# satoken/ractip

Hardware: NVIDIA B200
Metric: shuffled pairs/sec, probability stage of --zscore=12 (McCaskill in/out x2 + unpaired windows x2 + two-strand McCaskill) (higher is better)
Workload: dtype f64

## Files before the change

### ractip_b200/csrc/mcc_band.h

```cpp
#ifndef RP_MCC_BAND_H
#define RP_MCC_BAND_H

#include "mcc_core.h"

namespace rp {

constexpr int BR = 8;
constexpr int BSLOTS = 32;
constexpr int NSLICE = 16;

struct SmallModel {
  double scale1, mlb1, expMLclosing, expMLintern, expTermAU, inv_expTermAU;
  double scale_small[10];
  double mmI[8][5][5], mmH[8][5][5], mmM[8][5][5], mmExt[8][5][5], mm1n[8][5][5];
  double dangle5[8][5], dangle3[8][5];
  const double* spw;
  int special_hp, pad;
};
constexpr int SM_DOUBLES = (int)((sizeof(SmallModel) + 7) / 8);

struct DiagDesc;
struct BandShared {
  int LDB, LD8;
  int NGP;
  double *TI, *T1, *TA;
  double* ipart;
  double *cI, *c1, *cA;
  double* G;
  double *gA, *g1;
  double* sIv;
  SmallModel* sm;
  DiagDesc* desc;
};
constexpr int GPACK = (MAXLOOP + 1) * (MAXLOOP + 2) / 2;
constexpr int DESC_DOUBLES = 4 * 6;

RP_HD int band_ldb(int n) { return ((n + 1 + 7) / 8) * 8; }
RP_HD int band_ngp(int n) { return (n + 7) / 8 + 3; }
#ifdef __CUDACC__
constexpr bool BAND_SHFL = true;
#else
constexpr bool BAND_SHFL = false;
#endif
RP_HD size_t band_part_doubles(int n, int T, bool shfl = BAND_SHFL) {
  const size_t a = shfl ? (size_t)2 * BAND * (32 - (BAND - 1)) * (T / 32) : (size_t)2 * BAND * T;
  const size_t b = (size_t)(NSLICE + 1) * BR * band_ngp(n);
  return a > b ? a : b;
}
RP_HD size_t band_shared_doubles(int n, int T, bool shfl = BAND_SHFL) {
  return band_part_doubles(n, T, shfl) + 128  + (size_t)3 * BSLOTS * band_ldb(n) + (size_t)3 * BR * band_ngp(n) +
         GPACK + 64 + (size_t)(n + 2) + SM_DOUBLES + DESC_DOUBLES + (size_t)(n + 2 + 7) / 8 + 2;
}
RP_HD size_t band_shared_bytes(int n, int T, bool shfl = BAND_SHFL) { return band_shared_doubles(n, T, shfl) * sizeof(double); }

RP_HD void carve_band(Shared& sh, BandShared& bs, void* base, int n, int T, bool shfl = BAND_SHFL) {
  sh.T = T;
  double* p = static_cast<double*>(base);
  sh.part = p; bs.ipart = p; p += band_part_doubles(n, T, shfl);
  sh.red = p; p += 128;
  bs.LDB = band_ldb(n); bs.LD8 = bs.LDB / 8; bs.NGP = band_ngp(n);
  bs.TI = p; p += (size_t)BSLOTS * bs.LDB;
  bs.T1 = p; p += (size_t)BSLOTS * bs.LDB;
  bs.TA = p; p += (size_t)BSLOTS * bs.LDB;
  bs.cI = p; p += (size_t)BR * bs.NGP;
  bs.c1 = p; p += (size_t)BR * bs.NGP;
  bs.cA = p; p += (size_t)BR * bs.NGP;
  bs.G = p; p += GPACK;
  bs.gA = p; p += 32;
  bs.g1 = p; p += 32;
  bs.sIv = p; p += n + 2;
  bs.sm = reinterpret_cast<SmallModel*>(p); p += SM_DOUBLES;
  bs.desc = reinterpret_cast<DiagDesc*>(p); p += DESC_DOUBLES;
  sh.S = reinterpret_cast<uint8_t*>(p);
  sh.grow = nullptr; sh.ghead_b = nullptr; sh.ghead_1 = nullptr;
}

RP_HD void load_band_weights(const DevModel& M, const BandShared& bs, int tid, int T) {
  for (int x = tid; x < GPACK; x += T) bs.G[x] = M.gpack[x];
  for (int s = tid; s < 32; s += T) { bs.gA[s] = M.gA[s]; bs.g1[s] = M.g1[s]; }
  SmallModel& S = *bs.sm;
  if (tid == 0) {
    S.scale1 = M.scale1; S.mlb1 = M.mlb1; S.expMLclosing = M.expMLclosing; S.expMLintern = M.expMLintern;
    S.expTermAU = M.expTermAU; S.inv_expTermAU = 1.0 / M.expTermAU;
    for (int k = 0; k < 10; k++) S.scale_small[k] = M.scale_small[k];
    S.spw = M.spw;
    S.special_hp = M.special_hp; S.pad = 0;
  }
  for (int x = tid; x < 200; x += T) {
    (&S.mmI[0][0][0])[x] = (&M.mmI[0][0][0])[x];
    (&S.mmH[0][0][0])[x] = (&M.mmH[0][0][0])[x];
    (&S.mmM[0][0][0])[x] = (&M.mmM[0][0][0])[x];
    (&S.mmExt[0][0][0])[x] = (&M.mmExt[0][0][0])[x];
    (&S.mm1n[0][0][0])[x] = (&M.mm1n[0][0][0])[x];
    if (x < 40) {
      (&S.dangle5[0][0])[x] = (&M.dangle5[0][0])[x];
      (&S.dangle3[0][0])[x] = (&M.dangle3[0][0])[x];
    }
  }
}

RP_HD int bidx(const BandShared& bs, int p) { return (p & 7) * bs.LD8 + (p >> 3); }
RP_HD double* brow(double* band, const BandShared& bs, int d) { return band + (size_t)(d & (BSLOTS - 1)) * bs.LDB; }

struct Segs {
  int b[4];
  int G[4];
};
RP_HD Segs make_segs(int n, int cp, int d, bool cross_only = false) {
  Segs s;
  const int C = n - d;
  s.b[0] = 1; s.b[3] = C + 1;
  if (cp <= 0) { s.b[1] = C + 1; s.b[2] = C + 1; }
  else {
    int b1 = cp - d, b2 = cp;
    if (b1 < 1) b1 = 1;
    if (b1 > C + 1) b1 = C + 1;
    if (b2 > C + 1) b2 = C + 1;
    if (b2 < b1) b2 = b1;
    s.b[1] = b1; s.b[2] = b2;
  }
  if (cross_only && cp > 0) { s.b[0] = s.b[1]; s.b[3] = s.b[2]; }
  s.G[0] = 0;
  for (int k = 0; k < 3; k++) s.G[k + 1] = s.G[k] + (s.b[k + 1] - s.b[k] + BR - 1) / BR;
  return s;
}
RP_HD int seg_slot(const Segs& s, const BandShared& bs, int i) {
  const int k = (i >= s.b[1]) + (i >= s.b[2]);
  const int o = i - s.b[k];
  return (o & (BR - 1)) * bs.NGP + s.G[k] + (o >> 3);
}

struct DiagDesc {
  Segs sg;
  int gsh, NB, nitems, t0;
};
constexpr int NDESC = 4;
static_assert(sizeof(DiagDesc) * NDESC <= DESC_DOUBLES * sizeof(double), "descriptor ring");
RP_HD void band_make_desc(DiagDesc& D, int n, int cp, int d, int T, bool cross_only = false) {
  D.sg = make_segs(n, cp, d, cross_only);
  const int NG = D.sg.G[3], cells = D.sg.b[3] - D.sg.b[0];
  D.gsh = NG <= 8 ? 3 : 4;
  const int GB = 1 << D.gsh;
  D.NB = (NG + GB - 1) >> D.gsh;
  D.nitems = NSLICE * D.NB;
  const int Cw = (cells + 1 + 31) & ~31;
  D.t0 = (D.nitems * GB + 2 * Cw <= T) ? Cw : 0;
}

#ifdef __CUDA_ARCH__
__device__ __forceinline__ double ldg_now(const double* p) {
  double v;
  asm volatile("ld.global.f64 %0, [%1];" : "=d"(v) : "l"(p));
  return v;
}
#else
inline double ldg_now(const double* p) { return *p; }
#endif
RP_HD double ldg_if(bool ok, const double* p, const double* safe, double dflt) {
  const double v = ldg_now(ok ? p : safe);
  return ok ? v : dflt;
}

#ifdef __CUDA_ARCH__
struct RingPtr { unsigned a; };
__device__ __forceinline__ RingPtr ring_ptr(const double* p) { RingPtr r; r.a = (unsigned)__cvta_generic_to_shared(p); return r; }
__device__ __forceinline__ double ring_ld(RingPtr base, int ix, unsigned x, unsigned span) {
  double v;
  asm volatile("{\n\t.reg .pred p;\n\tsetp.le.u32 p, %2, %3;\n\tmov.f64 %0, 0d0000000000000000;\n\t@p ld.shared.f64 %0, [%1];\n\t}"
               : "=d"(v) : "r"(base.a + (unsigned)(ix * 8)), "r"(x), "r"(span));
  return v;
}
__device__ __forceinline__ void ring_adv(RingPtr& p, int elems) { p.a += (unsigned)(elems * 8); }
__device__ __forceinline__ void keep_in_reg(int& v) { asm volatile("" : "+r"(v)); }
#else
struct RingPtr { const double* a; };
inline RingPtr ring_ptr(const double* p) { RingPtr r; r.a = p; return r; }
inline double ring_ld(RingPtr base, int ix, unsigned x, unsigned span) { return x <= span ? base.a[ix] : 0.; }
inline void ring_adv(RingPtr& p, int elems) { p.a += elems; }
inline void keep_in_reg(int&) {}
#endif

template <int SIGN>
RP_HD void interior_item(const BandShared& bs, int n, int cp, int d, const Segs& sg, int q, int g, double* tot) {
#pragma unroll
  for (int r = 0; r < BR; r++) tot[r] = 0.;
  const int k = (g >= sg.G[1]) + (g >= sg.G[2]);
  const int i0 = sg.b[k] + BR * (g - sg.G[k]);
  const int smax = SIGN > 0 ? (d - 6 < MAXLOOP ? d - 6 : MAXLOOP) : (n - 3 - d < MAXLOOP ? n - 3 - d : MAXLOOP);
  const double* fI = bs.cI + g;
  const double* f1 = bs.c1 + g;
  const double* fA = bs.cA + g;
  const int NGP = bs.NGP, LD8 = bs.LD8;
#pragma unroll 1
  for (int h = 0; h < 2; h++) {
    const int s = h == 0 ? q : MAXLOOP - q;
    if (h == 1 && s == q) break;
    if (s > smax || s < 2) continue;
    const int dr = d - SIGN * (2 + s);
    const int P0 = SIGN > 0 ? i0 + 1 : i0 - 1 - s;
    int plo = 1, phi = n - dr;
    if (cp > 0) {
      if (SIGN > 0) {
        if (k == 1) { if (cp - dr > plo) plo = cp - dr; if (cp - 1 < phi) phi = cp - 1; }
      } else {
        if (k == 0) { if (cp - 1 - dr < phi) phi = cp - 1 - dr; }
        else if (k == 2) { if (cp > plo) plo = cp; }
      }
    }
    if (phi < plo) continue;
    const int clo = plo - P0;
    const unsigned span = (unsigned)(phi - plo);
    const int b = P0 & 7;
    const size_t ro = (size_t)(dr & (BSLOTS - 1)) * bs.LDB;
    const RingPtr rI = ring_ptr(bs.TI + ro + (P0 >> 3));
    const RingPtr r1 = ring_ptr(bs.T1 + ro + (P0 >> 3));
    const RingPtr rA = ring_ptr(bs.TA + ro + (P0 >> 3));
#define RP_IX(e) (((e) & 7) * LD8 + ((e) >> 3))
#pragma unroll 1
    for (int tb = 0; tb < (s >= 4 ? 2 : 1); tb++) {
      const RingPtr rp = tb ? r1 : rA;
      const double* f = tb ? f1 : fA;
      const double w = tb ? bs.g1[s] : bs.gA[s];
      const int eL = tb, eR = s - tb;
      const unsigned xl = (unsigned)(eL - clo), xr = (unsigned)(eR - clo);
#pragma unroll
      for (int r = 0; r < BR; r++) {
        const double x0 = ring_ld(rp, RP_IX(b + eL + r), xl + r, span), x1 = ring_ld(rp, RP_IX(b + eR + r), xr + r, span);
        tot[r] += f[r * NGP] * (w * (x0 + x1));
      }
    }
    if (s >= 6) {
      double acc[BR], win[BR];
#pragma unroll
      for (int r = 0; r < BR; r++) acc[r] = 0.;
#pragma unroll
      for (int r = 0; r < BR - 1; r++) win[r] = ring_ld(rI, RP_IX(b + 2 + r), (unsigned)(2 + r - clo), span);
      win[BR - 1] = 0.;
      int off[BR];
#pragma unroll
      for (int u = 0; u < BR; u++) { off[u] = RP_IX(b + 9 + u); keep_in_reg(off[u]); }
      const double* gw = bs.G + s * (s + 1) / 2 + 2;
      RingPtr pI = rI;
      unsigned cm = (unsigned)(9 - clo);
      const int nst = s - 3;
      int x = 0;
#pragma unroll 1
      for (; x + BR <= nst; x += BR) {
#pragma unroll
        for (int u = 0; u < BR; u++) {
          win[(u + BR - 1) & (BR - 1)] = ring_ld(pI, off[u], cm + u, span);
          const double gv = gw[u];
#pragma unroll
          for (int r = 0; r < BR; r++) acc[r] += gv * win[(u + r) & (BR - 1)];
        }
        ring_adv(pI, 1); cm += BR; gw += BR;
      }
#pragma unroll
      for (int u = 0; u < BR - 1; u++) {
        if (x + u < nst) {
          win[(u + BR - 1) & (BR - 1)] = ring_ld(pI, off[u], cm + u, span);
          const double gv = gw[u];
#pragma unroll
          for (int r = 0; r < BR; r++) acc[r] += gv * win[(u + r) & (BR - 1)];
        }
      }
#pragma unroll
      for (int r = 0; r < BR; r++) tot[r] += fI[r * NGP] * acc[r];
    }
#undef RP_IX
  }
}

RP_HD constexpr int sp_u1(int s) { return s == 0 ? 0 : s == 1 ? 1 : s == 2 ? 0 : s == 3 ? 1 : s == 4 ? 1 : s == 5 ? 2 : s == 6 ? 2 : s == 7 ? 2 : 3; }
RP_HD constexpr int sp_u2(int s) { return s == 0 ? 0 : s == 1 ? 0 : s == 2 ? 1 : s == 3 ? 1 : s == 4 ? 2 : s == 5 ? 1 : s == 6 ? 2 : s == 7 ? 3 : 2; }

RP_HD double band_plain(const BandShared& bs, int d, int p, int type) {
  const double v = bs.TA[(size_t)(d & (BSLOTS - 1)) * bs.LDB + bidx(bs, p)];
  return type > 2 ? v * bs.sm->inv_expTermAU : v;
}

template <class C>
RP_HD double inside_specials_band(const C& c, const BandShared& bs, int d, int i) {
  const SmallModel& M = *bs.sm;
  const int j = i + d;
  const int type = pair_type(base(c, i), base(c, j));
  const int ddmax = d - (TURN + 1) < MAXLOOP + 2 ? d - (TURN + 1) : MAXLOOP + 2;
  if (!type || ddmax < 2) return 0.;
  const int maxpo = (c.cp > 0 && i < c.cp) ? c.cp - 1 - i : 1000;
  const int maxu2 = (c.cp > 0 && j >= c.cp) ? j - 1 - c.cp : 1000;
  const int si1 = base(c, i + 1), sj1 = base(c, j - 1);
  double v[RP_N_SPECIAL], w[RP_N_SPECIAL];
#pragma unroll
  for (int s = 0; s < RP_N_SPECIAL; s++) {
    const int u1 = sp_u1(s), u2 = sp_u2(s), dd = u1 + u2 + 2;
    const bool ok = dd <= ddmax && u1 + 1 <= maxpo && u2 <= maxu2;
    const int k = ok ? i + 1 + u1 : i + 1, l = ok ? j - 1 - u2 : j - 1, dr = ok ? d - dd : d - 2;
    const int t2 = pair_type(base(c, k), base(c, l));
    v[s] = (ok && t2) ? band_plain(bs, dr, k, t2) : 0.;
    w[s] = special_loop(M, s, type, rtype(t2), si1, sj1, base(c, k - 1), base(c, l + 1));
// ... 324 lines not shown
```

### ractip_b200/csrc/mcc_band_shfl.cuh

```cuda
#ifndef RP_MCC_BAND_SHFL_CUH
#define RP_MCC_BAND_SHFL_CUH

#include "mcc_core.h"

namespace rp {

__device__ __forceinline__ double shfl_down_f64(double v, int delta) { return __shfl_down_sync(0xffffffffu, v, delta); }
__device__ __forceinline__ void prefetch_l2(const void* p) {
#ifdef __CUDA_ARCH__
  asm volatile("prefetch.global.L2 [%0];" ::"l"(p));
#else
  (void)p;
#endif
}
#define RP_MARK(k)                                                                                       \
  do {                                                                                                   \
    if (RP_PROF(c) && tid == 0) {                                                                            \
      const long long now__ = clock64();                                                                 \
      atomicAdd(reinterpret_cast<unsigned long long*>(RP_PROF(c) + (k)), (unsigned long long)(now__ - tmark)); \
      atomicAdd(reinterpret_cast<unsigned long long*>(RP_PROF(c) + 32 + (k)), 1ull);                         \
      tmark = clock64();                                                                                 \
    }                                                                                                    \
  } while (0)

constexpr int HW = 32 - (BAND - 1);
struct SplitW {
  int W;
  int S;
  int CP;
};
__device__ __forceinline__ SplitW make_split_w(int C, int T) {
  SplitW s;
  s.W = (C + HW - 1) / HW;
  s.S = (T / 32) / s.W;
  if (s.S < 1) s.S = 1;
  s.CP = s.W * HW;
  return s;
}

template <int NB = 4>
__device__ __forceinline__ void inside_band_A_shfl(const Ctx& c, const Shared& sh, int d0, int i0, int C, int tid) {
  const int T = sh.T;
  const SplitW sp = make_split_w(C, T);
  const int warp = tid >> 5, lane = tid & 31;
  const int slice = warp / sp.W, S = sp.S;
  if (slice >= S) return;
  const int cell = (warp - slice * sp.W) * HW + lane;
  const bool own = lane < HW && cell < C;
  const int i = i0 + cell;
  const bool rowok = i <= c.n - d0;
  const int ds = c.dstep();
  double m[BAND], q[BAND];
#pragma unroll
  for (int e = 0; e < BAND; e++) m[e] = q[e] = 0.;
  long long tmark = (RP_PROF(c) && tid == 0) ? clock64() : 0;
  if (!(RP_DBG(c) & 2)) {
    const int amax = d0 - 1;
    const int lim = d0 - TURN - 2;
    const int askip = c.cp > 0 ? c.cp - 1 - i : -1;
    const long es = ds;
    if (own) {
      for (int a = slice; a <= TURN && a <= amax; a += S) {
        const double A = TB(c, T_Q, a, i);
        const double* B = c.ptr(T_QQ, d0 - 1 - a, i + 1 + a);
        const int emin = a - lim;
#pragma unroll
        for (int e = 0; e < BAND; e++)
          if (e >= emin && e <= a) q[e] += A * B[e * es];
      }
    }
    RP_MARK(26);
    const int len = lim - TURN;
    if (len > 0) {
      const int per = (len + S - 1) / S;
      const int a_lo = TURN + 1 + slice * per;
      int a_hi = a_lo + per - 1;
      if (a_hi > lim) a_hi = lim;
      double bm[BAND], bq[BAND];
#pragma unroll
      for (int e = 0; e < BAND; e++) bm[e] = bq[e] = 0.;
      if (a_lo <= a_hi && rowok) {
        const double* Bm = c.ptr(T_QM1, d0 - 1 - a_lo, i + 1 + a_lo);
        const double* Bq = c.ptr(T_QQ, d0 - 1 - a_lo, i + 1 + a_lo);
#pragma unroll
        for (int e = 1; e < BAND; e++) { bm[e] = Bm[e * es]; bq[e] = Bq[e * es]; }
      }
      bool first = true;
#pragma unroll 1
      for (int a = a_lo; a <= a_hi; a += NB) {
        double Am[NB], Aq[NB], b0m[NB], b0q[NB];
#pragma unroll
        for (int u = 0; u < NB; u++) {
          const int au = a + u;
          const bool on = au <= a_hi;
          Am[u] = (on && own && au != askip) ? TB(c, T_QM, au, i) : 0.;
          Aq[u] = (on && own) ? TB(c, T_Q, au, i) : 0.;
          b0m[u] = (on && rowok) ? TB(c, T_QM1, d0 - 1 - au, i + 1 + au) : 0.;
          b0q[u] = (on && rowok) ? TB(c, T_QQ, d0 - 1 - au, i + 1 + au) : 0.;
        }
#pragma unroll
        for (int u = 0; u < NB; u++) {
          if (a + u <= a_hi) {
            if (!first) {
#pragma unroll
              for (int e = BAND - 1; e >= 1; e--) {
                bm[e] = shfl_down_f64(bm[e - 1], 1);
                bq[e] = shfl_down_f64(bq[e - 1], 1);
              }
            }
            first = false;
            bm[0] = b0m[u];
            bq[0] = b0q[u];
#pragma unroll
            for (int e = 0; e < BAND; e++) { m[e] += Am[u] * bm[e]; q[e] += Aq[u] * bq[e]; }
          }
        }
      }
    }
    RP_MARK(27);
    if (own) {
      const int a0 = lim + 1 > TURN + 1 ? lim + 1 : TURN + 1;
      for (int a = a0 + slice; a <= amax; a += S) {
        const double Am = (a == askip) ? 0. : TB(c, T_QM, a, i);
        const double Aq = TB(c, T_Q, a, i);
        const double* Bm = c.ptr(T_QM1, d0 - 1 - a, i + 1 + a);
        const double* Bq = c.ptr(T_QQ, d0 - 1 - a, i + 1 + a);
        const int emin = a - lim;
#pragma unroll
        for (int e = 0; e < BAND; e++)
          if (e >= emin) { m[e] += Am * Bm[e * es]; q[e] += Aq * Bq[e * es]; }
      }
    }
  }
  RP_MARK(28);
  if (!own) return;
#pragma unroll
  for (int e = 0; e < BAND; e++) {
    sh.part[((size_t)e * S + slice) * sp.CP + cell] = m[e];
    sh.part[((size_t)(BAND + e) * S + slice) * sp.CP + cell] = q[e];
  }
}
__device__ __forceinline__ void inside_band_B_shfl(Ctx& c, const Shared& sh, int d0, int i0, int C, int tid) {
  const int T = sh.T;
  const SplitW sp = make_split_w(C, T);
  for (int x = tid; x < BAND * C; x += T) {
    const int e = x / C, cell = x % C, i = i0 + cell;
    if (i + d0 + e > c.n) continue;
    double m = 0., q = 0.;
    for (int s = 0; s < sp.S; s++) {
      m += sh.part[((size_t)e * sp.S + s) * sp.CP + cell];
      q += sh.part[((size_t)(BAND + e) * sp.S + s) * sp.CP + cell];
    }
    TB(c, T_QM2, d0 + e, i) = m;
    TB(c, T_QS, d0 + e, i) = q;
  }
// ... 19 lines not shown
      const int l = d0 - BAND + 2 + r, k0 = l - d0;
      if (own && l <= n) {
#pragma unroll
        for (int e = 0; e < BAND; e++) {
          const int k = k0 + e, d = d0 - e;
          if (k > 2 && d > TURN) prefetch_l2(c.ptr(T_QB, d, k));
        }
      }
    }
    {
      const int k = 1 + r;
      const int tmax = n - k - d0 - (TURN + 3);
      int ecell = k + d0 - n;
      if (ecell < 0) ecell = 0;
      const long es = ds - ps;
      if (own) {
        for (int t = -(BAND - 1) + slice; t < 0 && t <= tmax; t += S) {
          const double A = TB(c, T_MC, d0 + TURN + 3 + t, k);
          const double* B = c.ptr(T_QM, TURN + 1 + t, k + d0 + 1);
          const int emin = -t > ecell ? -t : ecell;
#pragma unroll
          for (int e = 0; e < BAND; e++)
            if (e >= emin) pr[e] += A * B[e * es];
        }
      }
      const int tmax0 = __shfl_sync(0xffffffffu, tmax, 0);
      const bool pr_live = c.cp <= 0 || 1 + r0 + (warp - slice * sp.W) * HW < c.cp;
      if (tmax0 >= 0 && pr_live) {
        const int per = (tmax0 + 1 + S - 1) / S;
        const int t_lo = slice * per;
        int t_hi = t_lo + per - 1;
        if (t_hi > tmax0) t_hi = tmax0;
        double bv[BAND];
#pragma unroll
        for (int e = 0; e < BAND; e++) bv[e] = 0.;
        if (t_lo <= t_hi && t_lo <= tmax) {
          const double* B = c.ptr(T_QM, TURN + 1 + t_lo, k + d0 + 1);
#pragma unroll
          for (int e = 0; e < BAND - 1; e++) bv[e] = B[e * es];
        }
        bool first = true;
#pragma unroll 1
        for (int t = t_lo; t <= t_hi; t += NB) {
          double A[NB], b4[NB];
#pragma unroll
          for (int u = 0; u < NB; u++) {
            const int tu = t + u;
            const bool on = tu <= t_hi && tu <= tmax;
            A[u] = (on && own) ? TB(c, T_MC, d0 + TURN + 3 + tu, k) : 0.;
            b4[u] = on ? *(c.ptr(T_QM, TURN + 1 + tu, k + d0 + 1) + (BAND - 1) * es) : 0.;
          }
#pragma unroll
          for (int u = 0; u < NB; u++) {
            if (t + u <= t_hi) {
              if (!first) {
#pragma unroll
                for (int e = 0; e < BAND - 1; e++) bv[e] = shfl_down_f64(bv[e + 1], 1);
              }
              first = false;
              bv[BAND - 1] = b4[u];
#pragma unroll
              for (int e = 0; e < BAND; e++)
                if (e >= ecell) pr[e] += A[u] * bv[e];
            }
          }
        }
      }
    }
    RP_MARK(29);
    {
      const int l = d0 - BAND + 2 + r, k0 = l - d0;
      unsigned need = 0;
      if (own && l <= n) {
        double qbv[BAND];
        bool cand[BAND];
#pragma unroll
        for (int e = 0; e < BAND; e++) {
          const int k = k0 + e, d = d0 - e;
          cand[e] = k > 2 && d > TURN && pair_type(base(c, k), base(c, l)) != 0 && (c.cp <= 0 || (k < c.cp && l >= c.cp));
          qbv[e] = cand[e] ? TB(c, T_QB, d, k) : 0.;
        }
#pragma unroll
        for (int e = 0; e < BAND; e++)
          if (cand[e] && qbv[e] != 0.) need |= 1u << e;
      }
      RP_MARK(30);
      const int imax = k0 + (BAND - 1) - TURN - 3, imain = k0 - TURN - 3;
      const int imain_hi = __shfl_sync(0xffffffffu, imain, HW - 1);
      const bool ml_live = c.cp <= 0 || d0 - BAND + 2 + r0 + (warp - slice * sp.W) * HW + HW - 1 >= c.cp;
#pragma unroll 1
      for (int i = 1 + slice; ml_live && i <= imain_hi; i += NB * S) {
        double A[NB], b0[NB];
#pragma unroll
        for (int u = 0; u < NB; u++) {
          const int iu = i + u * S;
          const int row0 = k0 - 2 - iu;
          A[u] = (need != 0 && iu <= imain) ? TB(c, T_PRML, l - iu, iu) : 0.;
          b0[u] = (iu <= imain_hi && row0 >= 0 && k0 - 1 <= n) ? *(c.ptr(T_QM, 0, iu + 1) + (long)row0 * ds) : 0.;
        }
#pragma unroll
        for (int u = 0; u < NB; u++) {
          double bv[BAND];
          bv[0] = b0[u];
#pragma unroll
          for (int e = 1; e < BAND; e++) bv[e] = shfl_down_f64(b0[u], e);
#pragma unroll
          for (int e = 0; e < BAND; e++)
            if ((need >> e) & 1) ml[e] += A[u] * bv[e];
        }
      }
      if (need) {
        const int it0 = imain + 1 > 1 ? imain + 1 : 1;
        for (int i = it0 + slice; i <= imax; i += S) {
          const double A = TB(c, T_PRML, l - i, i);
          const double* B = c.ptr(T_QM, 0, i + 1) + (long)(k0 - 2 - i) * ds;
          const int emin = i - k0 + TURN + 3;
#pragma unroll
          for (int e = 0; e < BAND; e++)
            if (e >= emin && ((need >> e) & 1)) ml[e] += A * B[(long)e * ds];
        }
      }
    }
  }
  RP_MARK(31);
  if (!own) return;
#pragma unroll
  for (int e = 0; e < BAND; e++) {
    sh.part[((size_t)e * S + slice) * sp.CP + cell] = pr[e];
    sh.part[((size_t)(BAND + e) * S + slice) * sp.CP + cell] = ml[e];
  }
}
__device__ __forceinline__ void outside_band_B_shfl(Ctx& c, const Shared& sh, int d0, int r0, int C, int tid) {
  const int T = sh.T, n = c.n;
  const bool keep = c.kind == KIND_LINEAR && c.max_w > 0;
  const SplitW sp = make_split_w(C, T);
  for (int x = tid; x < BAND * C; x += T) {
    const int e = x / C, cell = x % C, r = r0 + cell, d = d0 - e;
    if (d < 1) continue;
    double a = 0., b = 0.;
    for (int s = 0; s < sp.S; s++) {
      a += sh.part[((size_t)e * sp.S + s) * sp.CP + cell];
      b += sh.part[((size_t)(BAND + e) * sp.S + s) * sp.CP + cell];
    }
    const int k = 1 + r;
    if (k + d <= n) {
      TB(c, T_PRB, d, k) = a;
      if (keep) RP_ST_STREAM(TB(c, T_XX, d, k), a);
    }
    const int l = d0 - BAND + 2 + r, k2 = l - d;
    if (l <= n && k2 >= 1) TB(c, T_MLB, d, k2) = b;
  }
}

}
#endif
```

### ractip_b200/csrc/mcc_driver.h

```cpp
#ifndef RP_MCC_DRIVER_H
#define RP_MCC_DRIVER_H

#include <type_traits>

#include "mcc_band.h"
#include "mcc_core.h"
#if defined(__CUDACC__) || defined(RP_HOST_SHFL)
#define RP_SHFL_FORMS 1
#include "mcc_band_shfl.cuh"
#include "mcc_wide_shfl.cuh"
#endif

namespace rp {

enum {
  PH_STAGE = 0, PH_PROLOGUE, PH_PROLOGUE2, PH_INSIDE_A, PH_INSIDE_B, PH_GENERIC_IN, PH_GENERIC_OUT, PH_OUTSIDE_A, PH_OUTSIDE_B,
  PH_WRITE_BP, PH_UN_ITEMS, PH_UN_DOMROWS, PH_UN_DOMCOLS, PH_UN_WINDOWS,
  PH_WRITE_HP, PH_LOGZ, PH_BAND_A, PH_BAND_B, PH_CFAC, PH_COUNT
};

template <class Exec, class = void>
struct CtasOf { static constexpr int value = 1; };
template <class Exec>
struct CtasOf<Exec, std::void_t<decltype(Exec::kCtas)>> { static constexpr int value = Exec::kCtas; };
// ... 97 lines not shown
        else wide_outside_A_shfl<W, WIDE_NB>(c, sh, d, r0, C, tid);
#else
        static_assert(!ShflOf<Exec>::value, "the shuffle forms are not compiled in");
#endif
      } else {
        if constexpr (W == BAND) outside_band_A(c, sh, d, r0, C, tid);
        else wide_outside_A<W>(c, sh, d, r0, C, tid);
      }
    });
    ex.phase(PH_BAND_B, [&](int tid) {
      if constexpr (ShflOf<Exec>::value) {
#ifdef RP_SHFL_FORMS
        if constexpr (W == BAND) outside_band_B_shfl(c, sh, d, r0, C, tid);
        else wide_outside_B_shfl<W>(c, sh, d, r0, C, tid);
#else
        static_assert(!ShflOf<Exec>::value, "the shuffle forms are not compiled in");
#endif
      } else {
        if constexpr (W == BAND) outside_band_B(c, sh, d, r0, C, tid);
        else wide_outside_B<W>(c, sh, d, r0, C, tid);
      }
    });
  });
}

template <class Exec, class MT>
RP_HD void emit_unpaired(Exec& ex, Ctx& c, const Problem& p, float* dense, const MT& SM, const double* gfull) {
  flat(ex, PH_UN_ITEMS, [&](int, int gt, int GT) { unstru_items(c, SM, gfull, gt, GT); });
  flat(ex, PH_UN_DOMROWS, [&](int, int gt, int GT) { unstru_dom_rows(c, gt, GT); });
  flat(ex, PH_UN_DOMCOLS, [&](int, int gt, int GT) { unstru_dom_cols(c, gt, GT); });
  if (p.out_up >= 0) flat(ex, PH_UN_WINDOWS, [&](int, int gt, int GT) { unstru_windows(c, dense + p.out_up, gt, GT); });
}

template <class Exec, class MT>
RP_HD void emit_outputs(Exec& ex, Ctx& c, const Problem& p, float* dense, const MT& SM, const double* gfull) {
  if (p.kind == KIND_LINEAR) {
    if (p.out_bp >= 0) {
      flat(ex, PH_WRITE_BP, [&](int, int gt, int GT) { write_bp(c, dense + p.out_bp, gt, GT); });
      flat(ex, PH_WRITE_BP, [&](int, int gt, int GT) { write_bp2(c, dense + p.out_bp, gt, GT); });
    }
    if (p.max_w > 0 && !p.defer_up) emit_unpaired(ex, c, p, dense, SM, gfull);
  } else if (p.kind == KIND_COFOLD) {
    if (p.out_hp >= 0)
      flat(ex, PH_WRITE_HP, [&](int, int gt, int GT) { write_hp(c, dense + p.out_hp, p.n1, p.n2, p.th_hy, gt, GT); });
  }
}

template <class Exec>
RP_HD void solve_mcc(Exec& ex, Ctx& c, const Problem& p, float* dense, double* logz, const Shared& sh) {
  const int T = sh.T;
  const int n = c.n;
  if (n + 2 <= RP_SMEM_SEQ) stage_sequence(ex, c, sh.S, [](int) {});
  ex.phase(PH_PROLOGUE, [&](int tid) {
    load_shared_model(*c.M, sh, tid);
    prologue_vectors(c, tid, T);
    prologue_lists(c, tid, T);
  });
  ex.phase(PH_PROLOGUE2, [&](int tid) { prologue2(c, tid, T); });

  for (int d = TURN + 1; d <= n - 1; d++) {
    if (d == band_start_inside(d)) split_sums_inside<BAND>(ex, c, sh, d);
    const int cells = n - d;
    const int chunk = cells < T ? cells : T;
    for (int i0 = 1; i0 <= cells; i0 += chunk) {
      const int C = cells - i0 + 1 < chunk ? cells - i0 + 1 : chunk;
      ex.phase(PH_INSIDE_A, [&](int tid) { inside_A(c, sh, d, i0, C, tid); });
      ex.phase(PH_INSIDE_B, [&](int tid) { inside_B(c, sh, d, i0, C, tid); });
    }
  }
  inside_end(c);
  emit_logz(ex, c, p, logz);

  for (int d = n - 1; d >= TURN + 1; d--) {
    if ((n - 1 - d) % BAND == 0) split_sums_outside<BAND>(ex, c, sh, d);
    const int lo = cross_lo(c, d), hi = cross_hi(c, d), cells = hi - lo + 1;
    const int chunk = cells < T ? cells : T;
    for (int i0 = lo; i0 <= hi; i0 += chunk) {
      const int C = hi - i0 + 1 < chunk ? hi - i0 + 1 : chunk;
      ex.phase(PH_OUTSIDE_A, [&](int tid) { outside_A(c, sh, d, i0, C, tid); });
      ex.phase(PH_OUTSIDE_B, [&](int tid) { outside_B(c, sh, d, i0, C, tid); });
    }
  }
  emit_outputs(ex, c, p, dense, *c.M, &c.M->gfull[0][0]);
}

template <class Exec>
RP_HD void solve_mcc_wide(Exec& ex, Ctx& c, const Problem& p, float* dense, double* logz, const Shared& sh) {
  constexpr int W = Exec::kWide;
  constexpr bool tile = CtasOf<Exec>::value == 1;
  const int T = sh.T;
  const int n = c.n;
  if (n + 2 <= RP_SMEM_SEQ) stage_sequence(ex, c, sh.S, [](int) {});
  flat(ex, PH_PROLOGUE, [&](int tid, int gt, int GT) {
    load_shared_model(*c.M, sh, tid);
    prologue_vectors(c, gt, GT);
    prologue_lists(c, gt, GT);
  });
  flat(ex, PH_PROLOGUE2, [&](int, int gt, int GT) {
    prologue2(c, gt, GT);
    prologue_rowmajor(c, gt, GT);
  });

  for (int d = TURN + 1; d <= n - 1; d++) {
    if (d == wide_start_inside<W>(d)) split_sums_inside<W>(ex, c, sh, d);
    const int cells = n - d;
    int sb[4] = {1, cells + 1, cells + 1, cells + 1};
    if (tile && c.cp > 0) {
      int b1 = c.cp - d, b2 = c.cp;
      if (b1 < 1) b1 = 1;
      if (b1 > cells + 1) b1 = cells + 1;
      if (b2 > cells + 1) b2 = cells + 1;
      if (b2 < b1) b2 = b1;
      sb[1] = b1; sb[2] = b2;
    }
    const bool staged = tile && W > BAND && gs_smax(n, d, 1) >= GS_ROW0;
    for (int sgm = 0; sgm < (tile ? 3 : 1); sgm++) {
      chunks(ex, sb[sgm], sb[sgm + 1], T, [&](int i0, int C) {
        const bool crossing = c.cp > 0 && sgm == 1;
        ex.phase(PH_INSIDE_A, [&](int tid) {
          if (staged) {
            stage_generic_tile<1>(c, sh, d, i0, C, crossing, tid);
            ends_items<1>(c, sh, d, i0, C, tid);
          } else {
            inside_A(c, sh, d, i0, C, tid);
          }
        });
        if (staged) ex.phase(PH_GENERIC_IN, [&](int tid) { generic_items<1>(c, sh, d, i0, C, tid); });
        ex.phase(PH_INSIDE_B, [&](int tid) { wide_inside_finish<W>(c, sh, d, i0, C, tid, staged); });
      });
    }
  }
  inside_end(c);
  emit_logz(ex, c, p, logz);

  for (int d = n - 1; d >= TURN + 1; d--) {
    if (d == wide_start_outside<W>(n, d)) split_sums_outside<W>(ex, c, sh, d);
    const bool staged = tile && W > BAND && gs_smax(n, d, -1) >= GS_ROW0;
    chunks(ex, cross_lo(c, d), cross_hi(c, d) + 1, T, [&](int i0, int C) {
      ex.phase(PH_OUTSIDE_A, [&](int tid) {
        if (staged) {
          stage_generic_tile<-1>(c, sh, d, i0, C, false, tid);
          ends_items<-1>(c, sh, d, i0, C, tid);
        } else {
          outside_A(c, sh, d, i0, C, tid);
        }
      });
      if (staged) ex.phase(PH_GENERIC_OUT, [&](int tid) { generic_items<-1>(c, sh, d, i0, C, tid); });
      ex.phase(PH_OUTSIDE_B, [&](int tid) { wide_outside_finish<W>(c, sh, d, i0, C, tid, staged); });
    });
  }
  emit_outputs(ex, c, p, dense, *c.M, &c.M->gfull[0][0]);
}

template <class Exec>
RP_HD const double* stage_gap_weights(Exec& ex, const Ctx& c, const BandShared& bs) {
  const double* gfull = &c.M->gfull[0][0];
  if ((size_t)3 * BSLOTS * bs.LDB < (size_t)(MAXLOOP + 1) * GROW_LD) return gfull;
  const int T = ex.nthreads();
  ex.phase(PH_STAGE, [&](int tid) {
    for (int x = tid; x < (MAXLOOP + 1) * GROW_LD; x += T) bs.TI[x] = gfull[x];
  });
  return bs.TI;
}

template <class Exec>
RP_HD void solve_band(Exec& ex, Ctx& c, const Problem& p, float* dense, double* logz, void* smem) {
  const int T = ex.nthreads();
  const int n = c.n;
  Shared sh;
  BandShared bs;
  carve_band(sh, bs, smem, n, T, ShflOf<Exec>::value);
  const bool wide = c.kind == KIND_LINEAR && c.max_w > 0;
  stage_sequence(ex, c, sh.S, [&](int tid) {
    load_band_weights(*c.M, bs, tid, T);
    prologue_vectors(c, tid, T);
  });
  ex.phase(PH_PROLOGUE2, [&](int tid) {
    prologue2(c, tid, T);
    if (tid == T - 1 && TURN + 1 <= n - 1) band_make_desc(bs.desc[(TURN + 1) & (NDESC - 1)], n, c.cp, TURN + 1, T);
  });

  ex.phase(PH_CFAC, [&](int tid) { band_collect<1>(c, bs, -1, TURN + 1 <= n - 1 ? TURN + 1 : -1, tid, T); });
  for (int d = TURN + 1; d <= n; d++) {
    const int dfin = d - 1 >= TURN + 1 ? d - 1 : -1;
    const int dnew = d <= n - 1 ? d : -1;
    ex.phase(PH_INSIDE_A, [&](int tid) {
      if (dfin >= 0) band_inside_B(c, sh, bs, dfin, wide, tid);
      if (dnew >= 0) band_interior_A<1>(c, bs, dnew, tid, T);
      if (tid == T - 1 && d + 1 <= n - 1) band_make_desc(bs.desc[(d + 1) & (NDESC - 1)], n, c.cp, d + 1, T);
    });
    if (dnew < 0) break;
    ex.phase(PH_CFAC, [&](int tid) { band_collect<1>(c, bs, dnew, d + 1 <= n - 1 ? d + 1 : -1, tid, T); });
    if (d == band_start_inside(d)) split_sums_inside<BAND>(ex, c, sh, d);
  }
  inside_end(c);
  emit_logz(ex, c, p, logz);

  if (n - 1 >= TURN + 1)
    ex.phase(PH_CFAC, [&](int tid) { if (tid == 0) band_make_desc(bs.desc[(n - 1) & (NDESC - 1)], n, c.cp, n - 1, T, true); });
  ex.phase(PH_CFAC, [&](int tid) { band_collect<-1>(c, bs, -1, n - 1 >= TURN + 1 ? n - 1 : -1, tid, T); });
  for (int d = n - 1; d >= TURN; d--) {
    const int dfin = d + 1 <= n - 1 ? d + 1 : -1;
    const int dnew = d >= TURN + 1 ? d : -1;
    if (dnew >= 0 && (n - 1 - d) % BAND == 0) split_sums_outside<BAND>(ex, c, sh, d);
    ex.phase(PH_OUTSIDE_A, [&](int tid) {
      if (dfin >= 0) band_outside_B(c, sh, bs, dfin, wide, tid);
      if (dnew >= 0) band_interior_A<-1>(c, bs, dnew, tid, T);
      if (tid == T - 1 && d - 1 >= TURN + 1) band_make_desc(bs.desc[(d - 1) & (NDESC - 1)], n, c.cp, d - 1, T, true);
    });
    if (dnew < 0) break;
    ex.phase(PH_CFAC, [&](int tid) {
      band_collect<-1>(c, bs, dnew, d - 1 >= TURN + 1 ? d - 1 : -1, tid, T);
    });
  }
  const double* gfull = wide && !p.defer_up ? stage_gap_weights(ex, c, bs) : &c.M->gfull[0][0];
  emit_outputs(ex, c, p, dense, *bs.sm, gfull);
}

template <class Exec>
RP_HD void solve_band_unpaired(Exec& ex, Ctx& c, const Problem& p, float* dense, void* smem) {
  const int T = ex.nthreads(), n = c.n;
  Shared sh;
  BandShared bs;
  carve_band(sh, bs, smem, n, T, ShflOf<Exec>::value);
  stage_sequence(ex, c, sh.S, [&](int tid) { load_band_weights(*c.M, bs, tid, T); });
  inside_end(c);
  emit_unpaired(ex, c, p, dense, *bs.sm, stage_gap_weights(ex, c, bs));
}

}
#endif
```

Measured before the change: 28680.

## Overlap far split-sum work with band diagonal steps using idle warps

Splits the band split-sum computation into a near part plus chunked far-range units that write partial sums to workspace slots. Warps left idle during each diagonal's interior phase are given far units ahead of time, tracked through new descriptor fields, so the later split phase only finishes the remaining units and reduces the slots. This aims to hide the periodic split-sum stalls behind the serial diagonal sweep. The cost is extra global workspace traffic for the partial sums, more descriptor state (the reduction scratch shrinks to make room), and a more complex schedule.

```diff
diff --git a/ractip_b200/csrc/mcc_band.h b/ractip_b200/csrc/mcc_band.h
--- a/ractip_b200/csrc/mcc_band.h
+++ b/ractip_b200/csrc/mcc_band.h
@@ -33,7 +33,8 @@
   DiagDesc* desc;
 };
 constexpr int GPACK = (MAXLOOP + 1) * (MAXLOOP + 2) / 2;
-constexpr int DESC_DOUBLES = 4 * 6;
+constexpr int DESC_DOUBLES = 4 * 8;
+constexpr int BAND_RED = 128 - (DESC_DOUBLES - 4 * 6);
 
 RP_HD int band_ldb(int n) { return ((n + 1 + 7) / 8) * 8; }
 RP_HD int band_ngp(int n) { return (n + 7) / 8 + 3; }
@@ -48,7 +49,7 @@
   return a > b ? a : b;
 }
 RP_HD size_t band_shared_doubles(int n, int T, bool shfl = BAND_SHFL) {
-  return band_part_doubles(n, T, shfl) + 128  + (size_t)3 * BSLOTS * band_ldb(n) + (size_t)3 * BR * band_ngp(n) +
+  return band_part_doubles(n, T, shfl) + BAND_RED + (size_t)3 * BSLOTS * band_ldb(n) + (size_t)3 * BR * band_ngp(n) +
          GPACK + 64 + (size_t)(n + 2) + SM_DOUBLES + DESC_DOUBLES + (size_t)(n + 2 + 7) / 8 + 2;
 }
 RP_HD size_t band_shared_bytes(int n, int T, bool shfl = BAND_SHFL) { return band_shared_doubles(n, T, shfl) * sizeof(double); }
@@ -57,7 +58,7 @@
   sh.T = T;
   double* p = static_cast<double*>(base);
   sh.part = p; bs.ipart = p; p += band_part_doubles(n, T, shfl);
-  sh.red = p; p += 128;
+  sh.red = p; p += BAND_RED;
   bs.LDB = band_ldb(n); bs.LD8 = bs.LDB / 8; bs.NGP = band_ngp(n);
   bs.TI = p; p += (size_t)BSLOTS * bs.LDB;
   bs.T1 = p; p += (size_t)BSLOTS * bs.LDB;
@@ -133,10 +134,21 @@
 struct DiagDesc {
   Segs sg;
   int gsh, NB, nitems, t0;
+  int far_w0, far_k, far_u, pad;
 };
 constexpr int NDESC = 4;
 static_assert(sizeof(DiagDesc) * NDESC <= DESC_DOUBLES * sizeof(double), "descriptor ring");
-RP_HD void band_make_desc(DiagDesc& D, int n, int cp, int d, int T, bool cross_only = false) {
+RP_HD int far_window_pos(int n, int d, bool outside) {
+  const int p = outside ? (n - 1 - d) % BAND : (d - TURN - 1) % BAND;
+  if (outside) return p - 1;
+  return p == 0 ? BAND - 2 : (p >= 2 ? p - 2 : -1);
+}
+RP_HD int far_window_band(int n, int d, bool outside) {
+  const int p = outside ? (n - 1 - d) % BAND : (d - TURN - 1) % BAND;
+  return outside ? d - BAND + p : (p == 0 ? d : d - p + BAND);
+}
+
+RP_HD void band_make_desc(DiagDesc& D, int n, int cp, int d, int T, bool cross_only = false, const DiagDesc* prev = nullptr) {
   D.sg = make_segs(n, cp, d, cross_only);
   const int NG = D.sg.G[3], cells = D.sg.b[3] - D.sg.b[0];
   D.gsh = NG <= 8 ? 3 : 4;
@@ -145,6 +157,17 @@
   D.nitems = NSLICE * D.NB;
   const int Cw = (cells + 1 + 31) & ~31;
   D.t0 = (D.nitems * GB + 2 * Cw <= T) ? Cw : 0;
+  int lo = n - d + 1;
+  if ((cross_only ? n - 3 - d : d - 6) >= 2) {
+    const int ie = D.t0 + D.nitems * GB;
+    if (ie > lo) lo = ie;
+  }
+  const int hi = T - (cells > 1 ? cells : 1);
+  const int pos = far_window_pos(n, d, cross_only);
+  D.far_w0 = (lo + 31) >> 5;
+  D.far_k = pos >= 0 && (hi >> 5) > D.far_w0 ? (hi >> 5) - D.far_w0 : 0;
+  D.far_u = pos > 0 && prev ? prev->far_u + prev->far_k : 0;
+  D.pad = 0;
 }
 
 #ifdef __CUDA_ARCH__
diff --git a/ractip_b200/csrc/mcc_band_shfl.cuh b/ractip_b200/csrc/mcc_band_shfl.cuh
--- a/ractip_b200/csrc/mcc_band_shfl.cuh
+++ b/ractip_b200/csrc/mcc_band_shfl.cuh
@@ -1,6 +1,7 @@
 #ifndef RP_MCC_BAND_SHFL_CUH
 #define RP_MCC_BAND_SHFL_CUH
 
+#include "mcc_band.h"
 #include "mcc_core.h"
 
 namespace rp {
@@ -326,5 +327,356 @@
   }
 }
 
+constexpr int FAR_STEPS = 8;
+constexpr int FAR_A0 = TURN + BAND;
+
+__device__ __forceinline__ double* split_slot(const Ctx& c, int s, int w, int e) {
+  return c.ws + ((unsigned)T_QMR * c.te + (unsigned)((s * 2 + w) * BAND + e) * (unsigned)c.ld);
+}
+
+struct SplitPlan {
+  int ngr, nf;
+};
+__device__ __forceinline__ int outside_pr_len(int n, int d0, int g) {
+  const int t = n - 1 - g * HW - d0 - (TURN + 3) + 1;
+  return t > 0 ? t : 0;
+}
+__device__ __forceinline__ int outside_ml_len(int n, int d0, int g) {
+  int rl = g * HW + HW - 1;
+  if (rl > n - d0 + BAND - 2) rl = n - d0 + BAND - 2;
+  const int i = rl - (BAND - 2) - (TURN + 3);
+  return i > 0 ? i : 0;
+}
+__device__ __forceinline__ SplitPlan band_split_plan(int n, int d0, bool outside) {
+  SplitPlan P;
+  int len;
+  if (!outside) {
+    P.ngr = n - d0 > 0 ? (n - d0 + HW - 1) / HW : 0;
+    len = d0 - TURN - 2 - FAR_A0 + 1;
+  } else {
+    P.ngr = (n - d0 + BAND - 1 + HW - 1) / HW;
+    len = 0;
+    for (int g = 0; g < P.ngr; g++) {
+      const int l = outside_pr_len(n, d0, g) + outside_ml_len(n, d0, g);
+      if (l > len) len = l;
+    }
+  }
+  P.nf = len > 0 ? (len + FAR_STEPS - 1) / FAR_STEPS : 0;
+  return P;
+}
+
+template <int NB>
+__device__ __forceinline__ void inside_split_unit(const Ctx& c, int d0, int g, int f, int lane) {
+  const int i = 1 + g * HW + lane;
+  const bool rowok = i <= c.n - d0;
+  const bool own = lane < HW && rowok;
+  const int ds = c.dstep();
+  const long es = ds;
+  const int amax = d0 - 1, lim = d0 - TURN - 2;
+  const int askip = c.cp > 0 ? c.cp - 1 - i : -1;
+  double m[BAND], q[BAND];
+#pragma unroll
+  for (int e = 0; e < BAND; e++) m[e] = q[e] = 0.;
+  int a_lo, a_hi;
+  if (f < 0) {
+    a_lo = TURN + 1;
+    a_hi = lim < FAR_A0 - 1 ? lim : FAR_A0 - 1;
+    if (own) {
+      double A[TURN + 1], B[TURN + 1][BAND];
+#pragma unroll
+      for (int a = 0; a <= TURN; a++) {
+        const bool on = a <= amax;
+        A[a] = on ? TB(c, T_Q, a, i) : 0.;
+#pragma unroll
+        for (int e = 0; e < BAND; e++) B[a][e] = (on && e >= a - lim && e <= a) ? TB(c, T_QQ, d0 - 1 - a + e, i + 1 + a) : 0.;
+      }
+#pragma unroll
+      for (int a = 0; a <= TURN; a++)
+#pragma unroll
+        for (int e = 0; e < BAND; e++) q[e] += A[a] * B[a][e];
+    }
+  } else {
+    a_lo = FAR_A0 + f * FAR_STEPS;
+    a_hi = a_lo + FAR_STEPS - 1 < lim ? a_lo + FAR_STEPS - 1 : lim;
+  }
+  double bm[BAND], bq[BAND];
+#pragma unroll
+  for (int e = 0; e < BAND; e++) bm[e] = bq[e] = 0.;
+  if (a_lo <= a_hi && rowok) {
+    const double* Bm = c.ptr(T_QM1, d0 - 1 - a_lo, i + 1 + a_lo);
+    const double* Bq = c.ptr(T_QQ, d0 - 1 - a_lo, i + 1 + a_lo);
+#pragma unroll
+    for (int e = 1; e < BAND; e++) { bm[e] = Bm[e * es]; bq[e] = Bq[e * es]; }
+  }
+  bool first = true;
+#pragma unroll 1
+  for (int a = a_lo; a <= a_hi; a += NB) {
+    double Am[NB], Aq[NB], b0m[NB], b0q[NB];
+#pragma unroll
+    for (int u = 0; u < NB; u++) {
+      const int au = a + u;
+      const bool on = au <= a_hi;
+      Am[u] = (on && own && au != askip) ? TB(c, T_QM, au, i) : 0.;
+      Aq[u] = (on && own) ? TB(c, T_Q, au, i) : 0.;
+      b0m[u] = (on && rowok) ? TB(c, T_QM1, d0 - 1 - au, i + 1 + au) : 0.;
+      b0q[u] = (on && rowok) ? TB(c, T_QQ, d0 - 1 - au, i + 1 + au) : 0.;
+    }
+#pragma unroll
+    for (int u = 0; u < NB; u++) {
+      if (a + u <= a_hi) {
+        if (!first) {
+#pragma unroll
+          for (int e = BAND - 1; e >= 1; e--) {
+            bm[e] = shfl_down_f64(bm[e - 1], 1);
+            bq[e] = shfl_down_f64(bq[e - 1], 1);
+          }
+        }
+        first = false;
+        bm[0] = b0m[u];
+        bq[0] = b0q[u];
+#pragma unroll
+        for (int e = 0; e < BAND; e++) { m[e] += Am[u] * bm[e]; q[e] += Aq[u] * bq[e]; }
+      }
+    }
+  }
+  if (f < 0 && own) {
+    const int a0 = lim + 1 > TURN + 1 ? lim + 1 : TURN + 1;
+#pragma unroll
+    for (int h = 0; h < TURN + 1; h += 2) {
+      double Am[2], Aq[2], Bm[2][BAND], Bq[2][BAND];
+#pragma unroll
+      for (int u = 0; u < 2; u++) {
+        const int a = a0 + h + u;
+        const bool on = a <= amax;
+        Am[u] = (on && a != askip) ? TB(c, T_QM, a, i) : 0.;
+        Aq[u] = on ? TB(c, T_Q, a, i) : 0.;
+#pragma unroll
+        for (int e = 0; e < BAND; e++) {
+          const bool ok = on && e >= a - lim;
+          Bm[u][e] = ok ? TB(c, T_QM1, d0 - 1 - a + e, i + 1 + a) : 0.;
+          Bq[u][e] = ok ? TB(c, T_QQ, d0 - 1 - a + e, i + 1 + a) : 0.;
+        }
+      }
+#pragma unroll
+      for (int u = 0; u < 2; u++)
+#pragma unroll
+        for (int e = 0; e < BAND; e++) { m[e] += Am[u] * Bm[u][e]; q[e] += Aq[u] * Bq[u][e]; }
+    }
+  }
+  if (!own) return;
+#pragma unroll
+  for (int e = 0; e < BAND; e++) {
+    split_slot(c, f + 1, 0, e)[i] = m[e];
+    split_slot(c, f + 1, 1, e)[i] = q[e];
+  }
+}
+
+template <int NB>
+__device__ __forceinline__ void outside_split_unit(const Ctx& c, int d0, int g, int f, int lane) {
+  const int n = c.n, ds = c.dstep(), ps = c.pstep();
+  const int r = g * HW + lane;
+  const bool own = lane < HW && r <= n - d0 + BAND - 2;
+  double pr[BAND], ml[BAND];
+#pragma unroll
+  for (int e = 0; e < BAND; e++) pr[e] = ml[e] = 0.;
+  const int k = 1 + r;
+  const int tmax = n - k - d0 - (TURN + 3);
+  const int ecell = k + d0 - n > 0 ? k + d0 - n : 0;
+  const long es = ds - ps;
+  const int l = d0 - BAND + 2 + r, k0 = l - d0;
+  const int imain = k0 - TURN - 3, imax = imain + BAND - 1;
+  const bool pr_live = c.cp <= 0 || 1 + g * HW < c.cp;
+  const bool ml_live = c.cp <= 0 || d0 - BAND + 2 + g * HW + HW - 1 >= c.cp;
+  int t_lo, t_hi, i_lo, i_hi;
+  if (f < 0) {
+    t_lo = 0; t_hi = -1; i_lo = 1; i_hi = 0;
+    if (own) {
+      double A[BAND - 1], B[BAND - 1][BAND];
+#pragma unroll
+      for (int h = 0; h < BAND - 1; h++) {
+        const int t = h - (BAND - 1);
+        const bool on = t <= tmax;
+        A[h] = on ? TB(c, T_MC, d0 + TURN + 3 + t, k) : 0.;
+#pragma unroll
+        for (int e = 0; e < BAND; e++)
+          B[h][e] = (on && e >= -t && e >= ecell) ? *(c.ptr(T_QM, TURN + 1 + t, k + d0 + 1) + e * es) : 0.;
+      }
+#pragma unroll
+      for (int h = 0; h < BAND - 1; h++)
+#pragma unroll
+        for (int e = 0; e < BAND; e++) pr[e] += A[h] * B[h][e];
+    }
+  } else {
+    const int P = outside_pr_len(n, d0, g), v_lo = f * FAR_STEPS, v_hi = v_lo + FAR_STEPS - 1;
+    t_lo = v_lo;
+    t_hi = v_hi < P - 1 ? v_hi : P - 1;
+    if (!pr_live) t_hi = -1;
+    const int L = outside_ml_len(n, d0, g);
+    i_lo = v_lo - P + 1 > 1 ? v_lo - P + 1 : 1;
+    i_hi = v_hi - P + 1 < L ? v_hi - P + 1 : L;
+    if (!ml_live) i_hi = 0;
+  }
+  if (t_lo <= t_hi) {
+    double bv[BAND];
+#pragma unroll
+    for (int e = 0; e < BAND; e++) bv[e] = 0.;
+    if (t_lo <= tmax) {
+      const double* B = c.ptr(T_QM, TURN + 1 + t_lo, k + d0 + 1);
+#pragma unroll
+      for (int e = 0; e < BAND - 1; e++) bv[e] = B[e * es];
+    }
+    bool first = true;
+#pragma unroll 1
+    for (int t = t_lo; t <= t_hi; t += NB) {
+      double A[NB], b4[NB];
+#pragma unroll
+      for (int u = 0; u < NB; u++) {
+        const int tu = t + u;
+        const bool on = tu <= t_hi && tu <= tmax;
+        A[u] = (on && own) ? TB(c, T_MC, d0 + TURN + 3 + tu, k) : 0.;
+        b4[u] = on ? *(c.ptr(T_QM, TURN + 1 + tu, k + d0 + 1) + (BAND - 1) * es) : 0.;
+      }
+#pragma unroll
+      for (int u = 0; u < NB; u++) {
+        if (t + u <= t_hi) {
+          if (!first) {
+#pragma unroll
+            for (int e = 0; e < BAND - 1; e++) bv[e] = shfl_down_f64(bv[e + 1], 1);
+          }
+          first = false;
+          bv[BAND - 1] = b4[u];
+#pragma unroll
+          for (int e = 0; e < BAND; e++)
+            if (e >= ecell) pr[e] += A[u] * bv[e];
+        }
+      }
+    }
+  }
+  unsigned need = 0;
+  if ((f < 0 || i_lo <= i_hi) && own && l <= n) {
+    double qbv[BAND];
+    bool cand[BAND];
+#pragma unroll
+    for (int e = 0; e < BAND; e++) {
+      const int kk = k0 + e, d = d0 - e;
+      cand[e] = kk > 2 && d > TURN && pair_type(base(c, kk), base(c, l)) != 0 && (c.cp <= 0 || (kk < c.cp && l >= c.cp));
+      qbv[e] = cand[e] ? TB(c, T_QB, d, kk) : 0.;
+    }
+#pragma unroll
+    for (int e = 0; e < BAND; e++)
+      if (cand[e] && qbv[e] != 0.) need |= 1u << e;
+  }
+#pragma unroll 1
+  for (int i = i_lo; i <= i_hi; i += NB) {
+    double A[NB], b0[NB];
+#pragma unroll
+    for (int u = 0; u < NB; u++) {
+      const int iu = i + u;
+      const int row0 = k0 - 2 - iu;
+      A[u] = (need != 0 && iu <= imain && iu <= i_hi) ? TB(c, T_PRML, l - iu, iu) : 0.;
+      b0[u] = (iu <= i_hi && row0 >= 0 && k0 - 1 <= n) ? *(c.ptr(T_QM, 0, iu + 1) + (long)row0 * ds) : 0.;
+    }
+#pragma unroll
+    for (int u = 0; u < NB; u++) {
+      double bv[BAND];
+      bv[0] = b0[u];
+#pragma unroll
+      for (int e = 1; e < BAND; e++) bv[e] = shfl_down_f64(b0[u], e);
+#pragma unroll
+      for (int e = 0; e < BAND; e++)
+        if ((need >> e) & 1) ml[e] += A[u] * bv[e];
+    }
+  }
+  if (f < 0 && need) {
+    const int it0 = imain + 1 > 1 ? imain + 1 : 1;
+    double A[BAND - 1], B[BAND - 1][BAND];
+#pragma unroll
+    for (int h = 0; h < BAND - 1; h++) {
+      const int i = it0 + h;
+      const bool on = i <= imax;
+      A[h] = on ? TB(c, T_PRML, l - i, i) : 0.;
+#pragma unroll
+      for (int e = 0; e < BAND; e++)
+        B[h][e] = (on && e >= i - k0 + TURN + 3 && ((need >> e) & 1)) ? *(c.ptr(T_QM, 0, i + 1) + (long)(k0 - 2 - i + e) * ds) : 0.;
+    }
+#pragma unroll
+    for (int h = 0; h < BAND - 1; h++)
+#pragma unroll
+      for (int e = 0; e < BAND; e++) ml[e] += A[h] * B[h][e];
+  }
+  if (!own) return;
+#pragma unroll
+  for (int e = 0; e < BAND; e++) {
+    split_slot(c, f + 1, 0, e)[r] = pr[e];
+    split_slot(c, f + 1, 1, e)[r] = ml[e];
+  }
+}
+
+template <int SIGN, int NB>
+__device__ __forceinline__ void split_unit(const Ctx& c, int d0, int g, int f, int lane) {
+  if (SIGN > 0) inside_split_unit<NB>(c, d0, g, f, lane);
+  else outside_split_unit<NB>(c, d0, g, f, lane);
+}
+
+template <int SIGN, int NB>
+__device__ __forceinline__ void band_far_units(const Ctx& c, const DiagDesc& D, int d, int tid) {
+  const int w = (tid >> 5) - D.far_w0;
+  if (w < 0 || w >= D.far_k) return;
+  const int d0 = far_window_band(c.n, d, SIGN < 0);
+  const SplitPlan P = band_split_plan(c.n, d0, SIGN < 0);
+  const int u = D.far_u + w;
+  if (u < P.ngr * P.nf) split_unit<SIGN, NB>(c, d0, u % P.ngr, u / P.ngr, tid & 31);
+}
+
+template <int SIGN, int NB>
+__device__ __forceinline__ void band_split_A(const Ctx& c, int d0, int done, int tid, int T) {
+  const SplitPlan P = band_split_plan(c.n, d0, SIGN < 0);
+  if (done > P.ngr * P.nf) done = P.ngr * P.nf;
+  const int nu = P.ngr + P.ngr * P.nf - done;
+  for (int x = tid >> 5; x < nu; x += T >> 5) {
+    const int u = x < P.ngr ? -1 : done + x - P.ngr;
+    split_unit<SIGN, NB>(c, d0, u < 0 ? x : u % P.ngr, u < 0 ? -1 : u / P.ngr, tid & 31);
+  }
+}
+
+__device__ __forceinline__ double split_sum(const Ctx& c, int nslot, int w, int e, int x) {
+  double s = split_slot(c, 0, w, e)[x];
+  int f = 1;
+  for (; f + 4 <= nslot; f += 4) {
+    double v[4];
+#pragma unroll
+    for (int u = 0; u < 4; u++) v[u] = split_slot(c, f + u, w, e)[x];
+#pragma unroll
+    for (int u = 0; u < 4; u++) s += v[u];
+  }
+  for (; f < nslot; f++) s += split_slot(c, f, w, e)[x];
+  return s;
+}
+__device__ __forceinline__ void inside_split_B(Ctx& c, int d0, int tid, int T) {
+  const int n = c.n, C = n - d0, nslot = 1 + band_split_plan(n, d0, false).nf;
+  for (int x = tid; x < BAND * C; x += T) {
+    const int e = x / C, i = 1 + x % C;
+    if (i + d0 + e > n) continue;
+    TB(c, T_QM2, d0 + e, i) = split_sum(c, nslot, 0, e, i);
+    TB(c, T_QS, d0 + e, i) = split_sum(c, nslot, 1, e, i);
+  }
+}
+__device__ __forceinline__ void outside_split_B(Ctx& c, int d0, int tid, int T) {
+  const int n = c.n, C = n - d0 + BAND - 1, nslot = 1 + band_split_plan(n, d0, true).nf;
+  const bool keep = c.kind == KIND_LINEAR && c.max_w > 0;
+  for (int x = tid; x < BAND * C; x += T) {
+    const int e = x / C, r = x % C, d = d0 - e;
+    if (d < 1) continue;
+    const int k = 1 + r;
+    if (k + d <= n) {
+      const double a = split_sum(c, nslot, 0, e, r);
+      TB(c, T_PRB, d, k) = a;
+      if (keep) RP_ST_STREAM(TB(c, T_XX, d, k), a);
+    }
+    const int l = d0 - BAND + 2 + r, k2 = l - d;
+    if (l <= n && k2 >= 1) TB(c, T_MLB, d, k2) = split_sum(c, nslot, 1, e, r);
+  }
+}
+
 }
 #endif
diff --git a/ractip_b200/csrc/mcc_driver.h b/ractip_b200/csrc/mcc_driver.h
--- a/ractip_b200/csrc/mcc_driver.h
+++ b/ractip_b200/csrc/mcc_driver.h
@@ -273,6 +273,38 @@
   emit_outputs(ex, c, p, dense, *c.M, &c.M->gfull[0][0]);
 }
 
+template <int SIGN, class Exec>
+RP_HD void band_split_sums(Exec& ex, Ctx& c, const Shared& sh, const BandShared& bs, int d0) {
+  if constexpr (ShflOf<Exec>::value) {
+#ifdef RP_SHFL_FORMS
+    const int T = ex.nthreads();
+    const int dl = SIGN > 0 ? d0 : d0 + 1;
+    const DiagDesc& D = bs.desc[dl & (NDESC - 1)];
+    const int done = dl <= c.n - 1 ? D.far_u + D.far_k : 0;
+    ex.phase(PH_BAND_A, [&](int tid) { band_split_A<SIGN, Exec::kBatch>(c, d0, done, tid, T); });
+    ex.phase(PH_BAND_B, [&](int tid) {
+      if constexpr (SIGN > 0) inside_split_B(c, d0, tid, T);
+      else outside_split_B(c, d0, tid, T);
+    });
+#else
+    static_assert(!ShflOf<Exec>::value, "the shuffle forms are not compiled in");
+#endif
+  } else if (SIGN > 0) {
+    split_sums_inside<BAND>(ex, c, sh, d0);
+  } else {
+    split_sums_outside<BAND>(ex, c, sh, d0);
+  }
+}
+
+template <int SIGN, class Exec>
+RP_HD void band_far_step(Exec&, const Ctx& c, const BandShared& bs, int d, int tid) {
+  if constexpr (ShflOf<Exec>::value) {
+#ifdef RP_SHFL_FORMS
+    band_far_units<SIGN, Exec::kBatch>(c, bs.desc[d & (NDESC - 1)], d, tid);
+#endif
+  }
+}
+
 template <class Exec>
 RP_HD const double* stage_gap_weights(Exec& ex, const Ctx& c, const BandShared& bs) {
   const double* gfull = &c.M->gfull[0][0];
@@ -307,12 +339,16 @@
     const int dnew = d <= n - 1 ? d : -1;
     ex.phase(PH_INSIDE_A, [&](int tid) {
       if (dfin >= 0) band_inside_B(c, sh, bs, dfin, wide, tid);
-      if (dnew >= 0) band_interior_A<1>(c, bs, dnew, tid, T);
-      if (tid == T - 1 && d + 1 <= n - 1) band_make_desc(bs.desc[(d + 1) & (NDESC - 1)], n, c.cp, d + 1, T);
+      if (dnew >= 0) {
+        band_interior_A<1>(c, bs, dnew, tid, T);
+        band_far_step<1>(ex, c, bs, dnew, tid);
+      }
+      if (tid == T - 1 && d + 1 <= n - 1)
+        band_make_desc(bs.desc[(d + 1) & (NDESC - 1)], n, c.cp, d + 1, T, false, &bs.desc[d & (NDESC - 1)]);
     });
     if (dnew < 0) break;
     ex.phase(PH_CFAC, [&](int tid) { band_collect<1>(c, bs, dnew, d + 1 <= n - 1 ? d + 1 : -1, tid, T); });
-    if (d == band_start_inside(d)) split_sums_inside<BAND>(ex, c, sh, d);
+    if (d == band_start_inside(d)) band_split_sums<1>(ex, c, sh, bs, d);
   }
   inside_end(c);
   emit_logz(ex, c, p, logz);
@@ -323,11 +359,15 @@
   for (int d = n - 1; d >= TURN; d--) {
     const int dfin = d + 1 <= n - 1 ? d + 1 : -1;
     const int dnew = d >= TURN + 1 ? d : -1;
-    if (dnew >= 0 && (n - 1 - d) % BAND == 0) split_sums_outside<BAND>(ex, c, sh, d);
+    if (dnew >= 0 && (n - 1 - d) % BAND == 0) band_split_sums<-1>(ex, c, sh, bs, d);
     ex.phase(PH_OUTSIDE_A, [&](int tid) {
       if (dfin >= 0) band_outside_B(c, sh, bs, dfin, wide, tid);
-      if (dnew >= 0) band_interior_A<-1>(c, bs, dnew, tid, T);
-      if (tid == T - 1 && d - 1 >= TURN + 1) band_make_desc(bs.desc[(d - 1) & (NDESC - 1)], n, c.cp, d - 1, T, true);
+      if (dnew >= 0) {
+        band_interior_A<-1>(c, bs, dnew, tid, T);
+        band_far_step<-1>(ex, c, bs, dnew, tid);
+      }
+      if (tid == T - 1 && d - 1 >= TURN + 1)
+        band_make_desc(bs.desc[(d - 1) & (NDESC - 1)], n, c.cp, d - 1, T, true, &bs.desc[d & (NDESC - 1)]);
     });
     if (dnew < 0) break;
     ex.phase(PH_CFAC, [&](int tid) {
```

Result: slower. 22760, median of 6 (-20.6%).
